# kakaoenterprise/JORLDY

Measured on NVIDIA H100. Metric: env_steps_per_sec, higher is better.
Workload: dtype f32

## Files before the change

include/jorldy_b200.h:

```cpp
#ifndef JORLDY_B200_H
#define JORLDY_B200_H

#include <stdint.h>

#ifdef __cplusplus
#define JB_API extern "C"
#else
#define JB_API
#endif

JB_API int jb_env_classic_reset(int kind, double* phys, float* obs, int32_t* elapsed, int64_t* episode,
                                float* score, const uint8_t* mask, uint64_t seed, uint64_t stream_base,
                                int n, void* stream);
JB_API int jb_env_classic_step(int kind, double* phys, float* obs, int32_t* elapsed, int64_t* episode,
                               float* score, const void* action, int action_kind, float* next_obs,
                               float* reward, float* done, float* stats, int auto_reset, int max_steps,
                               uint64_t seed, uint64_t stream_base, int n, void* stream);

JB_API int jb_gae(const float* reward, const float* done, const float* value, const float* next_value,
                  const float* last_value, int N, int T, float gamma, float lambda, int standardize,
                  float* adv, float* ret, void* stream);

JB_API int
jb_env_synth_reset(float* obs, int32_t* elapsed, int64_t* episode, float* score, uint64_t seed,
// ... 41 lines not shown
                            const float* relu_act, void* stream);
JB_API int jb_linear_bwd_dw(const float* dy, const float* x, float* dw, float* db, int M, int in_f, int out_f,
                            void* stream);
JB_API int
jb_linear_bwd_dw_splitk(const float* dy, const float* x, float* dw, float* db, int M, int in_f, int out_f,
                        float* workspace, int splits, void* stream);
JB_API int jb_linear_io_fwd(const float* x, const float* w, const float* b, float* y, int M, int in_f, int out_f,
                            int relu, void* stream);
JB_API int jb_linear_io_bwd_dx(const float* dy, const float* w, float* dx, int M, int in_f, int out_f,
                               const float* relu_act, void* stream);
JB_API int jb_linear_io_bwd_dw(const float* dy, const float* x, float* dw, int M, int in_f, int out_f, void* stream);
JB_API int jb_colsum(const float* x, int M, int N, float* out, int accumulate, void* stream);
JB_API int jb_mlp_in_fwd(const float* x, const int32_t* idx, const float* w1, const float* b1, int M, int D, int H,
                         float* h1, float* xg, void* stream);
JB_API int jb_heads_fwd(const float* h, int M, int H, const float* w0, const float* b0, int n0, const float* w1,
                        const float* b1, int n1, const float* w2, const float* b2, int n2, float* out, void* stream);
JB_API int jb_heads_bwd_dx(const float* dout, const float* h, int M, int H, const float* w0, int n0, const float* w1,
                           int n1, const float* w2, int n2, float* dh, void* stream);
JB_API int jb_heads_bwd_dw(const float* dout, const float* h, int M, int H, float* dw0, float* db0, int n0, float* dw1,
                           float* db1, int n1, float* dw2, float* db2, int n2, void* stream);

JB_API int jb_ppo_act_discrete(const float* out, int M, int A, int nout, const float* u, uint64_t seed,
                               uint64_t stream_base, uint64_t ctr, long long* row_ctr, int greedy, int64_t* action,
                               void* stream);
JB_API int jb_ppo_act_continuous(const float* out, int M, int A, int nout, const float* normal, uint64_t seed,
                                 uint64_t stream_base, uint64_t ctr, long long* row_ctr, int greedy, float* action,
                                 void* stream);
JB_API int jb_ppo_prepass_discrete(const float* out, const int32_t* action, int M, int A, int nout, float* value,
                                   float* logp_old, void* stream);
JB_API int jb_ppo_prepass_continuous(const float* out, const float* action, int M, int A, int nout, float* value,
                                     float* logp_old, void* stream);
JB_API int jb_take_minibatch(const int32_t* perm, long long* cursor, int B, int32_t* cur_idx, void* stream);
JB_API int jb_ppo_loss(int continuous, const float* out, const int32_t* idx, const void* action, const float* adv,
                       const float* ret, const float* value_old, const float* logp_old, int B, int A, int nout,
                       float eps_clip, float vf_coef, float ent_coef, float* dout, float* stats, float* acc,
                       void* stream);

JB_API int jb_env_frames_reset(uint8_t* obs, int64_t* fcount, float* score, uint64_t seed, uint64_t stream_base, int n,
                               void* stream);
JB_API int jb_env_frames_step(uint8_t* obs, int64_t* fcount, float* score, uint8_t* next_obs, float* reward, float* done,
// ... 103 lines not shown
```

jorldy_b200/core/agent/ppo.py:

```python
import numpy as np
import torch

from ..buffer import FrameRollout, RolloutBuffer
from ..dev import C, ptr, require_cuda, stream_ptr
from ..network import Network
from ..optimizer import Optimizer
from .base import BaseAgent

GRAPH_CHUNK = 16
MAX_ACTION_SIZE = {"discrete": 18, "continuous": 8}


class PPO(BaseAgent):
    def __init__(
        self,
        state_size,
        action_size,
        hidden_size=512,
        network="discrete_policy_value",
        head="mlp",
        optim_config={"name": "adam"},
        gamma=0.99,
        use_standardization=True,
        run_step=1e6,
# ... 45 lines not shown

        self.seed = int(seed)
        self.rng_stream_base = 0
        self._row_ctr = {}
        self.use_cuda_graph = use_cuda_graph
        self.use_fused = use_fused
        self._fused = {}
        self._graphs = {}
        self._acc = torch.zeros(8, dtype=torch.float32, device=self.device)
        self._cursor = torch.zeros(1, dtype=torch.int64, device=self.device)
        self.world_size = 1
        self.allreduce = None
        self._inject_perms = None
        self.n_launches = 0
        self.n_prepass_launches = 0

    @property
    def continuous(self):
        return self.action_type == "continuous"

    def act_device(self, state, training=True, noise=None):
        net = self.network
        M = state.shape[0]
        out = net._buf("act.out", (M, net.nout))
        net.forward_rows(state, out)
        A = self.action_size
        row_ctr = self._row_ctr.get(M)
        if row_ctr is None:
            row_ctr = self._row_ctr[M] = torch.zeros(M, dtype=torch.int64, device=self.device)
        if self.continuous:
            action = net._buf("act.a", (M, A))
            C.jb_ppo_act_continuous(ptr(out), M, A, net.nout, ptr(noise), self.seed, self.rng_stream_base,
                                    0, ptr(row_ctr), int(not training), ptr(action), stream_ptr())
        else:
            action = net._buf("act.a", (M,), torch.int64)
            C.jb_ppo_act_discrete(ptr(out), M, A, net.nout, ptr(noise), self.seed, self.rng_stream_base,
                                  0, ptr(row_ctr), int(not training), ptr(action), stream_ptr())
        return action

    @torch.no_grad()
    def act(self, state, training=True):
        self.network.train(training)
        s = self.as_tensor(state)
        action = self.act_device(s.view(s.shape[0], -1), training)
        a = action.cpu().numpy()
        return {"action": a.reshape(a.shape[0], -1)}

    def _minibatch_step(self, st, idx, B):
        net = self.network
        tag = f"mb{B}."
        out = net.forward_raw(st["state"], idx, B, tag=tag)
        dout = net._buf(tag + "dout", (B, net.nout))
        stats = net._buf(tag + "stats", (8 + 4 * ((B + 255) // 256),))
        C.jb_ppo_loss(int(self.continuous), ptr(out), ptr(idx), ptr(st["action"]), ptr(st["adv"]), ptr(st["ret"]),
                      ptr(st["value"]), ptr(st["logp_old"]), B, self.action_size, net.nout, self.epsilon_clip,
                      self.vf_coef, self.ent_coef, ptr(dout), ptr(stats), ptr(self._acc), stream_ptr())
        net.backward_raw(dout, B, tag=tag)
        if self.allreduce is not None:
            self.allreduce(net.grad)
        self.optimizer.step(max_norm=self.clip_grad_norm)

# ... 17 lines not shown
        side = torch.cuda.Stream()
        side.wait_stream(torch.cuda.current_stream())
        with torch.cuda.stream(side):
            C.jb_take_minibatch(ptr(st["perm"]), ptr(self._cursor), B, ptr(cur_idx), stream_ptr())
            self._minibatch_step(st, cur_idx, B)
        torch.cuda.current_stream().wait_stream(side)
        torch.cuda.synchronize()
        for dst, src in zip(mutated, saved):
            dst.copy_(src)
        graph = torch.cuda.CUDAGraph()
        with torch.cuda.graph(graph):
            chunk()
        self._graphs[key] = graph
        return graph

    def _learn_tensors(self, state, action, reward, done, next_state=None, last_next_state=None):
        net = self.network
        NT = state.shape[0]
        T = self.n_step
        N = NT // T
        assert N * T == NT, f"rollout of {NT} rows is not a multiple of n_step={T} (ppo.py:97 view(-1, n_step) would raise)"
        A = self.action_size
        dev = self.device
        s = stream_ptr()
        st = getattr(self, "_st", None)
        if st is None or st["NT"] != NT:
            st = {"NT": NT,
                  "out": torch.empty(NT, net.nout, device=dev),
                  "value": torch.empty(NT, device=dev),
                  "logp_old": torch.empty(NT, A if self.continuous else 1, device=dev),
                  "adv": torch.empty(NT, device=dev), "ret": torch.empty(NT, device=dev),
                  "next_value": torch.empty(NT, device=dev),
                  "perm": torch.empty(NT, dtype=torch.int32, device=dev)}
            self._st = st
        st["state"] = state
        st["action"] = action
        net.forward_rows(state, st["out"])
        if self.continuous:
            C.jb_ppo_prepass_continuous(ptr(st["out"]), ptr(action), NT, A, net.nout, ptr(st["value"]),
                                        ptr(st["logp_old"]), s)
        else:
            C.jb_ppo_prepass_discrete(ptr(st["out"]), ptr(action), NT, A, net.nout, ptr(st["value"]),
                                      ptr(st["logp_old"]), s)
        if next_state is not None:
            nout = net._buf("next.out", (NT, net.nout))
            net.forward_rows(next_state, nout)
            st["next_value"].copy_(nout[:, -1])
            nv, lv = st["next_value"], None
        else:
            lout = net._buf("last.out", (N, net.nout))
            net.forward_rows(last_next_state, lout)
            lv = net._buf("last.v", (N,))
            lv.copy_(lout[:, -1])
            nv = None
        C.jb_gae(ptr(reward), ptr(done), ptr(st["value"]), ptr(nv), ptr(lv), N, T, self.gamma, self._lambda,
                 int(self.use_standardization), ptr(st["adv"]), ptr(st["ret"]), s)
        mean_ret = st["ret"].mean()

        B = self.batch_size
        self.optimizer._sync_lr()
        self._acc.zero_()
        self._acc[3] = -float("inf")
        self._acc[4] = float("inf")
        n_full = NT // B
        tail = NT - n_full * B
        from . import ppo_fused
        use_fused = self.use_fused and n_full > 0 and ppo_fused.supported(self, B)
        if use_fused and B not in self._fused:
            self._fused[B] = ppo_fused.FusedRunner(self, B)
        use_graph = (not use_fused) and self.use_cuda_graph and n_full >= GRAPH_CHUNK
        n_steps = 0
        for epoch in range(self.n_epoch):
            if self._inject_perms is not None:
                perm = torch.as_tensor(np.asarray(self._inject_perms[epoch]), dtype=torch.int32, device=dev)
            else:
                perm = torch.randperm(NT, device=dev, dtype=torch.int32)
            st["perm"].copy_(perm)
            self._cursor.zero_()
            done_steps = 0
            if use_fused:
                self._fused[B].run(st, n_full)
                done_steps = n_full
            if use_graph:
                g = self._graph_for(st, B)
                for _ in range(n_full // GRAPH_CHUNK):
                    g.replay()
                done_steps = (n_full // GRAPH_CHUNK) * GRAPH_CHUNK
            for k in range(done_steps, n_full):
                self._minibatch_step(st, st["perm"][k * B:(k + 1) * B], B)
            if tail:
                self._minibatch_step(st, st["perm"][n_full * B:], tail)
            n_steps += n_full + (1 if tail else 0)
        self.n_launches = (self.n_epoch * (1 + (self.LAUNCHES_PER_MINIBATCH if tail else 0)) if use_fused
                           else n_steps * self.LAUNCHES_PER_MINIBATCH)
        n_chunks = (NT + 16383) // 16384
        self.n_prepass_launches = 3 * n_chunks + 1 + 3 + 1

        acc = torch.cat([self._acc[:6], mean_ret.view(1), self._acc[7:8]]).cpu().numpy()
        if acc[7] != 0.0:
            dbg = [ws["partials"][200:205].tolist() for ws in (r.ws for r in self._fused.values())]
            raise RuntimeError("persistent PPO kernel: a peer GPU did not reach the gradient exchange (flag wait timed out); "
                               f"[kind 1=grad-ready 2=done-reading, peer, step, seen, target] = {dbg}")
        cnt = max(acc[5], 1.0)
        return {
            "actor_loss": float(acc[0] / cnt),
            "critic_loss": float(acc[1] / cnt),
            "entropy_loss": float(acc[2] / cnt),
            "max_ratio": float(acc[3]),
            "min_prob": float(acc[4]),
            "mean_ret": float(acc[6]),
        }

    def _action_to_device(self, action):
# ... 18 lines not shown
            self._host_in = hin
        hin["state"].copy_(torch.as_tensor(tr["state"], dtype=torch.float32, device=dev).reshape(n, -1))
        hin["next_state"].copy_(torch.as_tensor(tr["next_state"], dtype=torch.float32, device=dev).reshape(n, -1))
        hin["reward"].copy_(torch.as_tensor(tr["reward"], dtype=torch.float32, device=dev).reshape(-1))
        hin["done"].copy_(torch.as_tensor(tr["done"], dtype=torch.float32, device=dev).reshape(-1))
        hin["action"].copy_(self._action_to_device(tr["action"]))
        return self._learn_tensors(hin["state"], hin["action"], hin["reward"], hin["done"], next_state=hin["next_state"])

    def learn_rollout(self, rollout):
        N, T = rollout.N, rollout.T
        frames = isinstance(rollout, FrameRollout)
        if frames:
            state, last = rollout.rows(), rollout.last_rows()
        else:
            state, last = rollout.state.view(N * T, -1), rollout.last_next_state
        res = self._learn_tensors(state, rollout.action.view(N * T, -1) if self.continuous
                                  else rollout.action.view(N * T), rollout.reward.view(N * T),
                                  rollout.done.view(N * T), last_next_state=last)
        if frames:
            rollout.frames.check()
        rollout.clear()
        return res

    def process(self, transitions, step):
        result = {}
        self.memory.store(transitions)
        delta_t = step - self.time_t
        self.time_t = step
        self.learn_stamp += delta_t
        if self.learn_stamp >= self.n_step:
            result = self.learn()
            if self.lr_decay:
                self.learning_rate_decay(step)
# ... 3 lines not shown
```

jorldy_b200/core/buffer/rollout_buffer.py:

```python
import numpy as np
import torch

from ..dev import require_cuda
from .base import BaseBuffer
from .frame_store import FrameRows, FrameStore, frames_per_rollout


class RolloutBuffer(BaseBuffer):
    def __init__(self):
        super().__init__()
        self.buffer = list()

    def store(self, transitions):
        if self.first_store:
            self.check_dim(transitions[0])
        self.buffer += transitions

    def sample(self):
        transitions = self.stack_transition(self.buffer)
        self.buffer.clear()
        return transitions

    def sample_batched(self):
        out = {}
        for key in self.buffer[0].keys():
            arr = np.stack([np.asarray(b[key]) for b in self.buffer], axis=1)
            out[key] = arr.reshape((-1,) + arr.shape[2:])
        self.buffer.clear()
        return out

    @property
    def size(self):
        return len(self.buffer)


class DeviceRollout:
    def __init__(self, num_envs, n_step, state_size, action_size, action_type, device=None):
        dev = require_cuda(device)
        N, T = num_envs, n_step
        self.N, self.T, self.device = N, T, dev
        self.state = torch.zeros(N, T, state_size, dtype=torch.float32, device=dev)
        if action_type == "discrete":
            self.action = torch.zeros(N, T, dtype=torch.int32, device=dev)
        else:
            self.action = torch.zeros(N, T, action_size, dtype=torch.float32, device=dev)
        self.reward = torch.zeros(N, T, dtype=torch.float32, device=dev)
        self.done = torch.zeros(N, T, dtype=torch.float32, device=dev)
        self.last_next_state = torch.zeros(N, state_size, dtype=torch.float32, device=dev)
        self.t = 0

    def write(self, state, action, reward, done, next_state):
        t = self.t
        self.state[:, t].copy_(state)
        if self.action.dtype == torch.int32:
            self.action[:, t].copy_(action.view(self.N))
        else:
# ... 10 lines not shown
            self.action[:, t].copy_(action.view(self.N))
        else:
            self.action[:, t].copy_(action.view(self.N, -1))
        self.reward[:, t].copy_(reward)
        self.done[:, t].copy_(done)
        if t == self.T - 1:
            self.last_next_state.copy_(next_state)
        self.t = t + 1

    @property
    def full(self):
        return self.t >= self.T

    def clear(self):
        self.t = 0


class FrameRollout(DeviceRollout):

    def __init__(self, num_envs, n_step, action_size, action_type, device=None):
        dev = require_cuda(device)
        N, T = num_envs, n_step
        self.N, self.T, self.device = N, T, dev
        self.frames = FrameStore(N, frames_per_rollout(T), dev)
        self.state_ref = torch.zeros(N, T, dtype=torch.int64, device=dev)
        if action_type == "discrete":
            self.action = torch.zeros(N, T, dtype=torch.int32, device=dev)
        else:
            self.action = torch.zeros(N, T, action_size, dtype=torch.float32, device=dev)
        self.reward = torch.zeros(N, T, dtype=torch.float32, device=dev)
        self.done = torch.zeros(N, T, dtype=torch.float32, device=dev)
        self.last_next_state = torch.zeros(N, dtype=torch.int64, device=dev)
        self._refs = torch.zeros(2, N, dtype=torch.int64, device=dev)
        self.t = 0

    def start(self, obs):
        self.frames.start(obs)

    def push(self, obs, next_obs, done, auto_reset):
        s, x = self.frames.push(obs, next_obs, done, auto_reset, out=self._refs)
        self.state_ref[:, self.t].copy_(s)
        return x

    def rows(self):
        return FrameRows(self.frames, self.state_ref.view(-1))

    def last_rows(self):
        return FrameRows(self.frames, self.last_next_state)
# ... 1 lines not shown
```

jorldy_b200/core/collect.py:

```python
import torch

from .buffer import DeviceRollout, FrameRollout, frame_store


class RolloutCollector:
    def __init__(self, env, agent, n_step=None, use_cuda_graph=True):
        self.env, self.agent = env, agent
        self.T = n_step or agent.n_step
        self.frames = bool(getattr(env, "frame_stack", False))
        if self.frames:
            self.rollout = FrameRollout(env.num_envs, self.T, env.action_size, env.action_type, device=agent.device)
        else:
            self.rollout = DeviceRollout(env.num_envs, self.T, env.state_size, env.action_size, env.action_type,
                                         device=agent.device)
        self.use_cuda_graph = use_cuda_graph
        self._graph = None
        self.launches_per_collect = 5 * self.T
        env.reset_device()
        if self.frames:
            self.rollout.start(env.obs)

    def _collect_eager(self):
        env, agent, ro = self.env, self.agent, self.rollout
        ro.clear()
        for t in range(self.T):
            if not self.frames:
                ro.state[:, t].copy_(env.obs)
            action = agent.act_device(env.obs, training=True)
            next_obs, reward, done = env.step_device(action)
            ro.t = t
            if self.frames:
                next_obs = ro.push(env.obs, next_obs, done, env.auto_reset)
            ro.write_after_step(action, reward, done, next_obs)

    def collect(self):
        if not self.use_cuda_graph:
            self._collect_eager()
            return self.rollout
        if self._graph is None:
            side = torch.cuda.Stream()
            side.wait_stream(torch.cuda.current_stream())
            with torch.cuda.stream(side):
                self._collect_eager()
            torch.cuda.current_stream().wait_stream(side)
            torch.cuda.synchronize()
            g = torch.cuda.CUDAGraph()
            with torch.cuda.graph(g):
                self._collect_eager()
            self._graph = g
        self._graph.replay()
        self.rollout.t = self.T
        return self.rollout


class NStepAssembler:

    def __init__(self, n_step, apex=False, gamma=0.99):
        self.n, self.apex, self.gamma = n_step, apex, gamma
        self.L = n_step + 1 if apex else n_step
        self.hist, self.count, self.pos = None, 0, 0

    def push(self, tr):
        if self.hist is None:
            self.hist = {k: torch.zeros((v.shape[0], self.L) + tuple(v.shape[1:]), dtype=v.dtype, device=v.device)
                         for k, v in tr.items()}
        for k, v in tr.items():
            self.hist[k][:, self.pos].copy_(v)
# ... 68 lines not shown
```

jorldy_b200/core/network/base.py:

```python
from collections import OrderedDict

import torch

from ..dev import C, ptr, require_cuda, stream_ptr

MAX_ROWS_PER_PASS = 16384


def orthogonal_(shape, gain, generator=None):
    w = torch.empty(shape, dtype=torch.float32)
    torch.nn.init.orthogonal_(w, gain, generator=generator)
    return w


def init_gain(nonlinearity):
    if isinstance(nonlinearity, str):
        if nonlinearity == "policy":
            return 0.01
        return torch.nn.init.calculate_gain(nonlinearity)
    return float(nonlinearity)


class _ParamList(list):
    network = None


class FlatNetwork:

    def __init__(self, device=None):
        self.device = require_cuda(device)
        self._specs = []
        self.training = True
        self._ws = {}

    def _allocate(self):
        total, offs = 0, []
        for _, shape in self._specs:
            n = 1
            for s in shape:
                n *= s
            offs.append(total)
            total += (n + 3) // 4 * 4
        self.num_flat = total
        self.flat = torch.zeros(total, dtype=torch.float32, device=self.device)
        self.grad = torch.zeros(total, dtype=torch.float32, device=self.device)
        self._offs = offs
        self.p = OrderedDict()
        self.g = OrderedDict()
# ... 22 lines not shown
        params = _ParamList(self.p.values())
        params.network = self
        return params

    def state_dict(self):
        return OrderedDict((k, v.detach().clone()) for k, v in self.p.items())

    def load_state_dict(self, sd):
        missing = [k for k in self.p if k not in sd]
        extra = [k for k in sd if k not in self.p]
        if missing or extra:
            raise KeyError(f"state_dict mismatch: missing {missing}, unexpected {extra}")
        with torch.no_grad():
            for k, v in self.p.items():
                v.copy_(torch.as_tensor(sd[k], dtype=torch.float32).to(self.device).view_as(v))

    def copy_from(self, other):
        assert other.num_flat == self.num_flat
        C.jb_copy_f32(ptr(self.flat), ptr(other.flat), self.num_flat, stream_ptr())

    def train(self, mode=True):
        self.training = mode
        return self

    def to(self, device):
        return self

    def _buf(self, key, shape, dtype=torch.float32):
        k = (key, tuple(shape), dtype)
        t = self._ws.get(k)
        if t is None:
            t = torch.empty(*shape, dtype=dtype, device=self.device)
            self._ws[k] = t
        return t
# ... 1 lines not shown
```

jorldy_b200/core/network/layers.py:

```python
from ..dev import C, ptr, stream_ptr


import os

TC_MIN_ROWS = 1024
_USE_TC = os.environ.get("JB_NO_TC", "0") != "1"


def linear_fwd(x, w, b, y, relu):
    M, in_f = x.shape
    out_f = w.shape[0]
    if _USE_TC and M >= TC_MIN_ROWS and M % 128 == 0 and out_f % 128 == 0 and in_f % 32 == 0 and b is not None:
        C.jb_linear_fwd_tc(ptr(x), ptr(w), ptr(b), ptr(y), M, in_f, out_f, int(relu), stream_ptr())
        return
    C.jb_linear_fwd(ptr(x), ptr(w), ptr(b), ptr(y), M, in_f, out_f, int(relu), stream_ptr())


def linear_bwd_dx(dy, w, dx, relu_act=None, accumulate=False):
    M, out_f = dy.shape
    in_f = w.shape[1]
    if accumulate:
        C.jb_gemm(ptr(dy), out_f, 1, ptr(w), in_f, 0, ptr(dx), in_f, M, in_f, out_f, 0, 0,
                  ptr(relu_act), in_f, 0, 1, stream_ptr())
    else:
        C.jb_linear_bwd_dx(ptr(dy), ptr(w), ptr(dx), M, in_f, out_f, ptr(relu_act), stream_ptr())


# ... 13 lines not shown
    if accumulate:
        C.jb_gemm(ptr(dy), out_f, 1, ptr(w), out_f, 1, ptr(dx), in_f, M, in_f, out_f, 0, 0,
                  ptr(relu_act), in_f, 0, 1, stream_ptr())
    else:
        C.jb_linear_io_bwd_dx(ptr(dy), ptr(w), ptr(dx), M, in_f, out_f, ptr(relu_act), stream_ptr())


def linear_io_bwd_dw(dy, x, dw, db):
    M, out_f = dy.shape
    C.jb_linear_io_bwd_dw(ptr(dy), ptr(x), ptr(dw), M, x.shape[1], out_f, stream_ptr())
    C.jb_colsum(ptr(dy), M, out_f, ptr(db), 0, stream_ptr())


def heads_fwd(h, heads, out):
    M, H = h.shape
    a = []
    for i in range(3):
        if i < len(heads):
            w, b = heads[i]
            a += [ptr(w), ptr(b), w.shape[0]]
        else:
            a += [0, 0, 0]
    C.jb_heads_fwd(ptr(h), M, H, *a, ptr(out), stream_ptr())


def heads_bwd_dx(dout, h, heads, dh):
    M, H = h.shape
    a = []
    for i in range(3):
        if i < len(heads):
            a += [ptr(heads[i][0]), heads[i][0].shape[0]]
        else:
            a += [0, 0]
    C.jb_heads_bwd_dx(ptr(dout), ptr(h), M, H, *a, ptr(dh), stream_ptr())


def heads_bwd_dw(dout, h, grads):
    M, H = h.shape
# ... 9 lines not shown
```

jorldy_b200/core/network/policy_value.py:

```python
import torch

from .base import FlatNetwork, init_gain, orthogonal_
from .head import make_head
from . import layers as L


class _PolicyValue(FlatNetwork):
    head_names = ()

    def __init__(self, D_in, D_out, D_hidden=512, head="mlp", device=None, seed=None):
        super().__init__(device)
        self.D_in, self.D_out, self.D_hidden = D_in, D_out, D_hidden
        self.head = make_head(head, D_in, D_hidden)
        self.out_heads = self._out_heads(D_out)
        self.nout = sum(n for _, n, _ in self.out_heads)
        self._wide = self.nout > 32
        assert not self._wide or len(self.out_heads) == 1
        specs = self.head.specs() + [("l.weight", (D_hidden, self.head.D_head_out)), ("l.bias", (D_hidden,))]
        for name, n, _ in self.out_heads:
            specs += [(f"{name}.weight", (n, D_hidden)), (f"{name}.bias", (n,))]
        self._specs = specs
        self._allocate()
        gen = torch.Generator().manual_seed(seed) if seed is not None else None
        with torch.no_grad():
# ... 17 lines not shown
            out = self._buf(tag + "out", (M, self.nout))
        if self._wide:
            w, b = self._heads_wb()[0]
            L.linear_fwd(h2, w, b, out, relu=False)
        else:
            L.heads_fwd(h2, self._heads_wb(), out)
        return out

    def forward_rows(self, x, out):
        M = x.shape[0]
        for s in range(0, M, self.head.max_rows):
            e = min(M, s + self.head.max_rows)
            self.forward_raw(x[s:e], None, e - s, out[s:e], tag=f"inf{e - s}.", save=False)
        return out

    def backward_raw(self, dout, M, tag="t."):
        h1 = self._buf(tag + "head.h", (M, self.head.D_head_out))
        h2 = self._buf(tag + "h2", (M, self.D_hidden))
        dh2 = self._buf(tag + "dh2", (M, self.D_hidden))
        dh1 = self._buf(tag + "dh1", (M, self.head.D_head_out))
        if self._wide:
            (w, _), (dw, db) = self._heads_wb()[0], self._heads_grads()[0]
            L.linear_bwd_dw(dout, h2, dw, db)
            L.linear_bwd_dx(dout, w, dh2, relu_act=h2)
        else:
            L.heads_bwd_dw(dout, h2, self._heads_grads())
            L.heads_bwd_dx(dout, h2, self._heads_wb(), dh2)
        L.linear_bwd_dw(dh2, h1, self.g["l.weight"], self.g["l.bias"])
        L.linear_bwd_dx(dh2, self.p["l.weight"], dh1, relu_act=h1)
        self.head.backward(self, dh1, M, tag)
# ... 23 lines not shown
```

jorldy_b200/core/optimizer/__init__.py:

```python
from collections import OrderedDict

import numpy as np
import torch

from ..dev import C, ptr, stream_ptr


class _FlatOptimizer:
    def __init__(self, params, lr):
        net = getattr(params, "network", None)
        if net is None:
            raise TypeError("jorldy_b200 optimizers take `params=network.parameters()` of a FlatNetwork")
        self.network = net
        self.defaults = {"lr": lr}
        self.param_groups = [{"lr": lr, "params": list(range(len(net.p)))}]
        dev = net.device
        self._lr_dev = torch.tensor([lr], dtype=torch.float32, device=dev)
        self._lr_host = float(lr)
        self._step_dev = torch.zeros(1, dtype=torch.int64, device=dev)
        self._n_partials = C.jb_grad_partials_count(net.num_flat)
        self._partials = torch.zeros(self._n_partials, dtype=torch.float32, device=dev)
        self.grad_norm = torch.zeros(1, dtype=torch.float32, device=dev)

    def _sync_lr(self):
# ... 21 lines not shown

    def __init__(self, params, lr=1e-3, betas=(0.9, 0.999), eps=1e-8, **kwargs):
        super().__init__(params, lr)
        self.betas, self.eps = betas, eps
        self.exp_avg = torch.zeros_like(self.network.flat)
        self.exp_avg_sq = torch.zeros_like(self.network.flat)

    def step(self, max_norm=None):
        self._sync_lr()
        net, s = self.network, stream_ptr()
        C.jb_grad_sumsq(ptr(net.grad), net.num_flat, ptr(self._partials), ptr(self._step_dev), s)
        C.jb_adam_step(ptr(net.flat), ptr(net.grad), ptr(self.exp_avg), ptr(self.exp_avg_sq), net.num_flat,
                       ptr(self._lr_dev), self.betas[0], self.betas[1], self.eps, ptr(self._step_dev),
                       ptr(self._partials), self._n_partials, float(max_norm) if max_norm else 0.0,
                       ptr(self.grad_norm), s)

    def state_dict(self):
        step = float(self._step_dev.item())
        m, v = self._slot_views(self.exp_avg), self._slot_views(self.exp_avg_sq)
        state = {i: {"step": torch.tensor(step), "exp_avg": m[i].clone(), "exp_avg_sq": v[i].clone()}
                 for i in range(len(m))} if step > 0 else {}
        group = {"lr": float(self.param_groups[0]["lr"]), "betas": self.betas, "eps": self.eps, "weight_decay": 0,
                 "amsgrad": False, "params": list(range(len(m)))}
        return {"state": state, "param_groups": [group]}

    def load_state_dict(self, sd):
        g = sd["param_groups"][0]
        self.param_groups[0]["lr"] = float(g["lr"])
        st = sd.get("state", {})
        if st:
# ... 12 lines not shown
    def __init__(self, params, lr=1e-2, alpha=0.99, eps=1e-8, centered=False, **kwargs):
        super().__init__(params, lr)
        if not centered:
            raise NotImplementedError("only RMSprop(centered=True) is on the hot path (config/ape_x/*.py)")
        self.alpha, self.eps, self.centered = alpha, eps, centered
        self.square_avg = torch.zeros_like(self.network.flat)
        self.grad_avg = torch.zeros_like(self.network.flat)

    def step(self, max_norm=None):
        self._sync_lr()
        net, s = self.network, stream_ptr()
        C.jb_grad_sumsq(ptr(net.grad), net.num_flat, ptr(self._partials), ptr(self._step_dev), s)
        C.jb_rmsprop_centered_step(ptr(net.flat), ptr(net.grad), ptr(self.square_avg), ptr(self.grad_avg),
                                   net.num_flat, ptr(self._lr_dev), self.alpha, self.eps, ptr(self._partials),
                                   self._n_partials, float(max_norm) if max_norm else 0.0, ptr(self.grad_norm), s)

    def state_dict(self):
        step = float(self._step_dev.item())
        sq, ga = self._slot_views(self.square_avg), self._slot_views(self.grad_avg)
        state = {i: {"step": torch.tensor(step), "square_avg": sq[i].clone(), "grad_avg": ga[i].clone()}
                 for i in range(len(sq))} if step > 0 else {}
        group = {"lr": float(self.param_groups[0]["lr"]), "alpha": self.alpha, "eps": self.eps, "centered": True,
                 "momentum": 0, "weight_decay": 0, "params": list(range(len(sq)))}
        return {"state": state, "param_groups": [group]}

    def load_state_dict(self, sd):
        self.param_groups[0]["lr"] = float(sd["param_groups"][0]["lr"])
        st = sd.get("state", {})
        if st:
            sq, ga = self._slot_views(self.square_avg), self._slot_views(self.grad_avg)
# ... 22 lines not shown
```

jorldy_b200/csrc/heads.cu:

```cuda
#include "common.cuh"

namespace {

constexpr int MAX_DIN = 32;
constexpr int MAX_NOUT = 32;

__global__ void mlp_in_fwd_kernel(const float* __restrict__ x, const int32_t* __restrict__ idx,
                                  const float* __restrict__ W1, const float* __restrict__ b1,
                                  int M, int D, int H, float* __restrict__ h1, float* __restrict__ xg) {
  const int m = blockIdx.y;
  const int j = blockIdx.x * blockDim.x + threadIdx.x;
  __shared__ float sx[MAX_DIN];
  const int row = idx ? idx[m] : m;
  if (threadIdx.x < D) {
    const float v = x[(size_t)row * D + threadIdx.x];
    sx[threadIdx.x] = v;
    if (xg && blockIdx.x == 0) xg[(size_t)m * D + threadIdx.x] = v;
  }
  __syncthreads();
  if (j >= H) return;
  float acc = 0.f;
  for (int i = 0; i < D; ++i) acc = fmaf(sx[i], W1[(size_t)j * D + i], acc);
  acc += b1[j];
  h1[(size_t)m * H + j] = fmaxf(acc, 0.f);
}

struct HeadRows {
  const float* w[MAX_NOUT];
  const float* b[MAX_NOUT];
};
struct HeadGradRows {
  float* dw[MAX_NOUT];
  float* db[MAX_NOUT];
};

__global__ void __launch_bounds__(256)
heads_fwd_kernel(const float* __restrict__ h, int M, int H, HeadRows hr, int nout, float* __restrict__ out) {
  const int warp = (blockIdx.x * blockDim.x + threadIdx.x) >> 5;
  const int lane = threadIdx.x & 31;
  if (warp >= M) return;
  float acc[MAX_NOUT];
#pragma unroll
  for (int o = 0; o < MAX_NOUT; ++o) acc[o] = 0.f;
  const float* hrow = h + (size_t)warp * H;
  int j = lane;
  for (; j + 96 < H; j += 128) {
    float hv[4];
#pragma unroll
    for (int u = 0; u < 4; ++u) hv[u] = hrow[j + 32 * u];
#pragma unroll
    for (int o = 0; o < MAX_NOUT; ++o) {
      if (o < nout) {
        float wv[4];
#pragma unroll
        for (int u = 0; u < 4; ++u) wv[u] = hr.w[o][j + 32 * u];
#pragma unroll
        for (int u = 0; u < 4; ++u) acc[o] = fmaf(hv[u], wv[u], acc[o]);
      }
    }
  }
  for (; j < H; j += 32) {
    const float hv = hrow[j];
#pragma unroll
    for (int o = 0; o < MAX_NOUT; ++o)
      if (o < nout) acc[o] = fmaf(hv, hr.w[o][j], acc[o]);
  }
#pragma unroll
  for (int o = 0; o < MAX_NOUT; ++o) {
    if (o < nout) {
      const float v = jb_warp_sum(acc[o]);
      if (lane == 0) out[(size_t)warp * nout + o] = v + *hr.b[o];
    }
  }
}

__global__ void heads_bwd_dx_kernel(const float* __restrict__ dout, const float* __restrict__ h, int M, int H,
                                    HeadRows hr, int nout, float* __restrict__ dh) {
  const int m = blockIdx.y;
  const int j = blockIdx.x * blockDim.x + threadIdx.x;
  __shared__ float sd[MAX_NOUT];
  if (threadIdx.x < nout) sd[threadIdx.x] = dout[(size_t)m * nout + threadIdx.x];
  __syncthreads();
  if (j >= H) return;
  float acc = 0.f;
#pragma unroll
  for (int o = 0; o < MAX_NOUT; ++o)
// ... 63 lines not shown
  for (int g = 0; g < 3; ++g)
    for (int q = 0; q < n[g]; ++q, ++o) {
      if (o >= MAX_NOUT || !w[g]) return false;
      hr.w[o] = w[g] + (size_t)q * H;
      hr.b[o] = b[g] ? b[g] + q : nullptr;
    }
  for (; o < MAX_NOUT; ++o) { hr.w[o] = nullptr; hr.b[o] = nullptr; }
  return true;
}

}

JB_API int jb_mlp_in_fwd(const float* x, const int32_t* idx, const float* w1, const float* b1, int M, int D, int H,
                         float* h1, float* xg, void* stream) {
  if (!x || !w1 || !b1 || !h1 || M <= 0 || D <= 0 || D > MAX_DIN || H <= 0) return JB_ERR_INVALID;
  dim3 grid(jb_div_up(H, 128), M);
  mlp_in_fwd_kernel<<<grid, 128, 0, (cudaStream_t)stream>>>(x, idx, w1, b1, M, D, H, h1, xg);
  return jb_check_launch();
}

JB_API int jb_heads_fwd(const float* h, int M, int H, const float* w0, const float* b0, int n0, const float* w1,
                        const float* b1, int n1, const float* w2, const float* b2, int n2, float* out, void* stream) {
  const int nout = n0 + n1 + n2;
  if (!h || !out || M <= 0 || H <= 0 || nout <= 0 || nout > MAX_NOUT) return JB_ERR_INVALID;
  const float* w[3] = {w0, w1, w2}; const float* b[3] = {b0, b1, b2}; const int n[3] = {n0, n1, n2};
  for (int g = 0; g < 3; ++g) if (n[g] > 0 && (!w[g] || !b[g])) return JB_ERR_INVALID;
  HeadRows hr;
  if (!fill_rows(hr, w, b, n, H)) return JB_ERR_INVALID;
  const int threads = 256;
  heads_fwd_kernel<<<jb_div_up((long long)M * 32, threads), threads, 0, (cudaStream_t)stream>>>(h, M, H, hr, nout, out);
  return jb_check_launch();
}

JB_API int jb_heads_bwd_dx(const float* dout, const float* h, int M, int H, const float* w0, int n0, const float* w1,
                           int n1, const float* w2, int n2, float* dh, void* stream) {
  const int nout = n0 + n1 + n2;
  if (!dout || !h || !dh || M <= 0 || H <= 0 || nout <= 0 || nout > MAX_NOUT) return JB_ERR_INVALID;
  const float* w[3] = {w0, w1, w2}; const float* b[3] = {nullptr, nullptr, nullptr}; const int n[3] = {n0, n1, n2};
  HeadRows hr;
  if (!fill_rows(hr, w, b, n, H)) return JB_ERR_INVALID;
  dim3 grid(jb_div_up(H, 128), M);
  heads_bwd_dx_kernel<<<grid, 128, 0, (cudaStream_t)stream>>>(dout, h, M, H, hr, nout, dh);
  return jb_check_launch();
}

// ... 18 lines not shown
```

jorldy_b200/csrc/ppo.cu:

```cuda
#include "common.cuh"
#include "philox.cuh"
#include "ppo_rowmath.cuh"

namespace {

using jbppo::MAX_A;
using jbppo::MAX_A_DISC;
using jbppo::log_softmax_row;
using jbppo::atanh_clamped;

template <int NA>
__global__ void ppo_act_discrete_kernel(const float* __restrict__ out, int M, int A, int nout,
                                        const float* __restrict__ u_in, uint64_t seed, uint64_t stream_base,
                                        uint64_t ctr, long long* __restrict__ row_ctr, int greedy,
                                        int64_t* __restrict__ action) {
  const int m = blockIdx.x * blockDim.x + threadIdx.x;
  if (m >= M) return;
  if (row_ctr) { ctr += (uint64_t)row_ctr[m]; row_ctr[m] += 1; }
  float lg[NA], lsm[NA];
#pragma unroll
  for (int a = 0; a < NA; ++a) lg[a] = a < A ? out[(size_t)m * nout + a] : 0.f;
  log_softmax_row<NA>(lg, A, lsm);
  int pick = 0;
  if (greedy) {
    float best = expf(lsm[0]);
#pragma unroll
    for (int a = 1; a < NA; ++a) if (a < A) { const float p = expf(lsm[a]); if (p > best) { best = p; pick = a; } }
  } else {
    float u;
    if (u_in) u = u_in[m];
    else { jb_philox4 r = jb_philox(seed, stream_base + (uint64_t)m, ctr); u = jb_u01_float(r.x); }
    float tot = 0.f;
#pragma unroll
    for (int a = 0; a < NA; ++a) if (a < A) tot += expf(lsm[a]);
    const float target = u * tot;
    float c = 0.f;
    bool found = false;
    pick = A - 1;
#pragma unroll
    for (int a = 0; a < NA; ++a) if (a < A && !found) { c += expf(lsm[a]); if (target < c) { pick = a; found = true; } }
  }
  action[m] = pick;
}

__global__ void ppo_act_continuous_kernel(const float* __restrict__ out, int M, int A, int nout,
                                          const float* __restrict__ n_in, uint64_t seed, uint64_t stream_base,
                                          uint64_t ctr, long long* __restrict__ row_ctr, int greedy,
                                          float* __restrict__ action) {
  const int m = blockIdx.x * blockDim.x + threadIdx.x;
  if (m >= M) return;
  if (row_ctr) { ctr += (uint64_t)row_ctr[m]; row_ctr[m] += 1; }
  for (int a = 0; a < A; a += 2) {
    float n0 = 0.f, n1 = 0.f;
    if (!greedy) {
      if (n_in) { n0 = n_in[(size_t)m * A + a]; if (a + 1 < A) n1 = n_in[(size_t)m * A + a + 1]; }
      else {
        jb_philox4 r = jb_philox(seed, stream_base + (uint64_t)m, ctr * 8 + (uint64_t)(a >> 1));
        const float u1 = (float)((r.x >> 8) + 1u) * (1.0f / 16777216.0f);
        const float u2 = jb_u01_float(r.y);
        const float rad = sqrtf(-2.0f * logf(u1));
        n0 = rad * cospif(2.0f * u2); n1 = rad * sinpif(2.0f * u2);
      }
    }
    for (int q = 0; q < 2 && a + q < A; ++q) {
      const float mu = fminf(fmaxf(out[(size_t)m * nout + a + q], -5.f), 5.f);
      const float sd = expf(tanhf(out[(size_t)m * nout + A + a + q]));
      const float z = greedy ? mu : fmaf(sd, q ? n1 : n0, mu);
      action[(size_t)m * A + a + q] = tanhf(z);
    }
  }
}

template <int NA>
__global__ void ppo_prepass_discrete_kernel(const float* __restrict__ out, const int32_t* __restrict__ action,
                                            int M, int A, int nout, float* __restrict__ value,
                                            float* __restrict__ logp_old) {
  const int m = blockIdx.x * blockDim.x + threadIdx.x;
  if (m >= M) return;
  float lg[NA], lsm[NA];
#pragma unroll
  for (int a = 0; a < NA; ++a) lg[a] = a < A ? out[(size_t)m * nout + a] : 0.f;
// ... 119 lines not shown
                                      int32_t* __restrict__ cur_idx) {
  const long long base = (*cursor) * (long long)B;
  for (int i = threadIdx.x; i < B; i += blockDim.x) cur_idx[i] = perm[base + i];
  __syncthreads();
  if (threadIdx.x == 0) *cursor += 1;
}

}

JB_API int jb_take_minibatch(const int32_t* perm, long long* cursor, int B, int32_t* cur_idx, void* stream) {
  if (!perm || !cursor || !cur_idx || B <= 0) return JB_ERR_INVALID;
  take_minibatch_kernel<<<1, 256, 0, (cudaStream_t)stream>>>(perm, cursor, B, cur_idx);
  return jb_check_launch();
}

JB_API int jb_ppo_act_discrete(const float* out, int M, int A, int nout, const float* u, uint64_t seed,
                               uint64_t stream_base, uint64_t ctr, long long* row_ctr, int greedy, int64_t* action,
                               void* stream) {
  if (!out || !action || M <= 0 || A <= 0 || A > MAX_A_DISC || nout < A) return JB_ERR_INVALID;
  const dim3 grid(jb_div_up(M, 128));
  cudaStream_t s = (cudaStream_t)stream;
  if (A <= MAX_A) ppo_act_discrete_kernel<MAX_A><<<grid, 128, 0, s>>>(out, M, A, nout, u, seed, stream_base, ctr, row_ctr, greedy, action);
  else ppo_act_discrete_kernel<MAX_A_DISC><<<grid, 128, 0, s>>>(out, M, A, nout, u, seed, stream_base, ctr, row_ctr, greedy, action);
  return jb_check_launch();
}

JB_API int jb_ppo_act_continuous(const float* out, int M, int A, int nout, const float* normal, uint64_t seed,
                                 uint64_t stream_base, uint64_t ctr, long long* row_ctr, int greedy, float* action,
                                 void* stream) {
  if (!out || !action || M <= 0 || A <= 0 || A > MAX_A || nout < 2 * A) return JB_ERR_INVALID;
  ppo_act_continuous_kernel<<<jb_div_up(M, 128), 128, 0, (cudaStream_t)stream>>>(out, M, A, nout, normal, seed, stream_base, ctr, row_ctr, greedy, action);
  return jb_check_launch();
}

JB_API int jb_ppo_prepass_discrete(const float* out, const int32_t* action, int M, int A, int nout, float* value,
                                   float* logp_old, void* stream) {
  if (!out || !action || !value || !logp_old || M <= 0 || A <= 0 || A > MAX_A_DISC || nout != A + 1) return JB_ERR_INVALID;
  const dim3 grid(jb_div_up(M, 128));
  cudaStream_t s = (cudaStream_t)stream;
  if (A <= MAX_A) ppo_prepass_discrete_kernel<MAX_A><<<grid, 128, 0, s>>>(out, action, M, A, nout, value, logp_old);
  else ppo_prepass_discrete_kernel<MAX_A_DISC><<<grid, 128, 0, s>>>(out, action, M, A, nout, value, logp_old);
  return jb_check_launch();
}

JB_API int jb_ppo_prepass_continuous(const float* out, const float* action, int M, int A, int nout, float* value,
                                     float* logp_old, void* stream) {
// ... 21 lines not shown
```

Baseline: 1.825 million.

## Reuse rollout policy outputs in PPO prepass and retile input/head kernels

During collection the policy outputs from acting are written straight into a rollout buffer through a strided output, and a network version counter records which weights produced them. At learn time, if the weights are unchanged and the row counts give bitwise-identical kernel paths, the prepass forward over all N*T states is skipped. The input-layer kernel now handles 16 rows per block with weights held in registers, and the heads kernel gains a 512-wide unrolled loop. The cost is extra rollout memory and version bookkeeping, and the reused outputs are only valid while the row-exactness check holds.

```diff
diff --git a/include/jorldy_b200.h b/include/jorldy_b200.h
--- a/include/jorldy_b200.h
+++ b/include/jorldy_b200.h
@@ -79,16 +79,17 @@
 JB_API int jb_mlp_in_fwd(const float* x, const int32_t* idx, const float* w1, const float* b1, int M, int D, int H,
                          float* h1, float* xg, void* stream);
 JB_API int jb_heads_fwd(const float* h, int M, int H, const float* w0, const float* b0, int n0, const float* w1,
-                        const float* b1, int n1, const float* w2, const float* b2, int n2, float* out, void* stream);
+                        const float* b1, int n1, const float* w2, const float* b2, int n2, float* out, int ldo,
+                        void* stream);
 JB_API int jb_heads_bwd_dx(const float* dout, const float* h, int M, int H, const float* w0, int n0, const float* w1,
                            int n1, const float* w2, int n2, float* dh, void* stream);
 JB_API int jb_heads_bwd_dw(const float* dout, const float* h, int M, int H, float* dw0, float* db0, int n0, float* dw1,
                            float* db1, int n1, float* dw2, float* db2, int n2, void* stream);
 
-JB_API int jb_ppo_act_discrete(const float* out, int M, int A, int nout, const float* u, uint64_t seed,
+JB_API int jb_ppo_act_discrete(const float* out, int M, int A, int ldo, const float* u, uint64_t seed,
                                uint64_t stream_base, uint64_t ctr, long long* row_ctr, int greedy, int64_t* action,
                                void* stream);
-JB_API int jb_ppo_act_continuous(const float* out, int M, int A, int nout, const float* normal, uint64_t seed,
+JB_API int jb_ppo_act_continuous(const float* out, int M, int A, int ldo, const float* normal, uint64_t seed,
                                  uint64_t stream_base, uint64_t ctr, long long* row_ctr, int greedy, float* action,
                                  void* stream);
 JB_API int jb_ppo_prepass_discrete(const float* out, const int32_t* action, int M, int A, int nout, float* value,
diff --git a/jorldy_b200/core/agent/ppo.py b/jorldy_b200/core/agent/ppo.py
--- a/jorldy_b200/core/agent/ppo.py
+++ b/jorldy_b200/core/agent/ppo.py
@@ -83,15 +83,17 @@
         self._inject_perms = None
         self.n_launches = 0
         self.n_prepass_launches = 0
+        self.timeline = None
 
     @property
     def continuous(self):
         return self.action_type == "continuous"
 
-    def act_device(self, state, training=True, noise=None):
+    def act_device(self, state, training=True, noise=None, out=None):
         net = self.network
         M = state.shape[0]
-        out = net._buf("act.out", (M, net.nout))
+        if out is None:
+            out = net._buf("act.out", (M, net.nout))
         net.forward_rows(state, out)
         A = self.action_size
         row_ctr = self._row_ctr.get(M)
@@ -99,11 +101,11 @@
             row_ctr = self._row_ctr[M] = torch.zeros(M, dtype=torch.int64, device=self.device)
         if self.continuous:
             action = net._buf("act.a", (M, A))
-            C.jb_ppo_act_continuous(ptr(out), M, A, net.nout, ptr(noise), self.seed, self.rng_stream_base,
+            C.jb_ppo_act_continuous(ptr(out), M, A, out.stride(0), ptr(noise), self.seed, self.rng_stream_base,
                                     0, ptr(row_ctr), int(not training), ptr(action), stream_ptr())
         else:
             action = net._buf("act.a", (M,), torch.int64)
-            C.jb_ppo_act_discrete(ptr(out), M, A, net.nout, ptr(noise), self.seed, self.rng_stream_base,
+            C.jb_ppo_act_discrete(ptr(out), M, A, out.stride(0), ptr(noise), self.seed, self.rng_stream_base,
                                   0, ptr(row_ctr), int(not training), ptr(action), stream_ptr())
         return action
 
@@ -114,6 +116,12 @@
         action = self.act_device(s.view(s.shape[0], -1), training)
         a = action.cpu().numpy()
         return {"action": a.reshape(a.shape[0], -1)}
+
+    def _mark(self, piece):
+        if self.timeline is not None:
+            ev = torch.cuda.Event(enable_timing=True)
+            ev.record()
+            self.timeline.append((piece, ev))
 
     def _minibatch_step(self, st, idx, B):
         net = self.network
@@ -161,7 +169,7 @@
         self._graphs[key] = graph
         return graph
 
-    def _learn_tensors(self, state, action, reward, done, next_state=None, last_next_state=None):
+    def _learn_tensors(self, state, action, reward, done, next_state=None, last_next_state=None, out=None):
         net = self.network
         NT = state.shape[0]
         T = self.n_step
@@ -182,12 +190,17 @@
             self._st = st
         st["state"] = state
         st["action"] = action
-        net.forward_rows(state, st["out"])
+        self._mark("start")
+        prepass_forward = out is None
+        if prepass_forward:
+            out = st["out"]
+            net.forward_rows(state, out)
+            self._mark("prepass_forward")
         if self.continuous:
-            C.jb_ppo_prepass_continuous(ptr(st["out"]), ptr(action), NT, A, net.nout, ptr(st["value"]),
+            C.jb_ppo_prepass_continuous(ptr(out), ptr(action), NT, A, net.nout, ptr(st["value"]),
                                         ptr(st["logp_old"]), s)
         else:
-            C.jb_ppo_prepass_discrete(ptr(st["out"]), ptr(action), NT, A, net.nout, ptr(st["value"]),
+            C.jb_ppo_prepass_discrete(ptr(out), ptr(action), NT, A, net.nout, ptr(st["value"]),
                                       ptr(st["logp_old"]), s)
         if next_state is not None:
             nout = net._buf("next.out", (NT, net.nout))
@@ -203,6 +216,7 @@
         C.jb_gae(ptr(reward), ptr(done), ptr(st["value"]), ptr(nv), ptr(lv), N, T, self.gamma, self._lambda,
                  int(self.use_standardization), ptr(st["adv"]), ptr(st["ret"]), s)
         mean_ret = st["ret"].mean()
+        self._mark("prepass_gae")
 
         B = self.batch_size
         self.optimizer._sync_lr()
@@ -224,6 +238,7 @@
                 perm = torch.randperm(NT, device=dev, dtype=torch.int32)
             st["perm"].copy_(perm)
             self._cursor.zero_()
+            self._mark("perm")
             done_steps = 0
             if use_fused:
                 self._fused[B].run(st, n_full)
@@ -238,12 +253,15 @@
             if tail:
                 self._minibatch_step(st, st["perm"][n_full * B:], tail)
             n_steps += n_full + (1 if tail else 0)
+            self._mark("epoch")
+        net.version += 1
         self.n_launches = (self.n_epoch * (1 + (self.LAUNCHES_PER_MINIBATCH if tail else 0)) if use_fused
                            else n_steps * self.LAUNCHES_PER_MINIBATCH)
-        n_chunks = (NT + 16383) // 16384
-        self.n_prepass_launches = 3 * n_chunks + 1 + 3 + 1
+        n_chunks = (NT + net.head.max_rows - 1) // net.head.max_rows
+        self.n_prepass_launches = 3 * n_chunks * prepass_forward + 1 + 3 + 1
 
         acc = torch.cat([self._acc[:6], mean_ret.view(1), self._acc[7:8]]).cpu().numpy()
+        self._mark("readback")
         if acc[7] != 0.0:
             dbg = [ws["partials"][200:205].tolist() for ws in (r.ws for r in self._fused.values())]
             raise RuntimeError("persistent PPO kernel: a peer GPU did not reach the gradient exchange (flag wait timed out); "
@@ -292,9 +310,14 @@
             state, last = rollout.rows(), rollout.last_rows()
         else:
             state, last = rollout.state.view(N * T, -1), rollout.last_next_state
+        net = self.network
+        out = None
+        if (rollout.out is not None and rollout.out_version == (net, net.version) and net.rows_exact(N)
+                and net.rows_exact(N * T)):
+            out = rollout.out.view(N * T, net.nout)
         res = self._learn_tensors(state, rollout.action.view(N * T, -1) if self.continuous
                                   else rollout.action.view(N * T), rollout.reward.view(N * T),
-                                  rollout.done.view(N * T), last_next_state=last)
+                                  rollout.done.view(N * T), last_next_state=last, out=out)
         if frames:
             rollout.frames.check()
         rollout.clear()
diff --git a/jorldy_b200/core/buffer/rollout_buffer.py b/jorldy_b200/core/buffer/rollout_buffer.py
--- a/jorldy_b200/core/buffer/rollout_buffer.py
+++ b/jorldy_b200/core/buffer/rollout_buffer.py
@@ -35,11 +35,13 @@
 
 
 class DeviceRollout:
-    def __init__(self, num_envs, n_step, state_size, action_size, action_type, device=None):
+    def __init__(self, num_envs, n_step, state_size, action_size, action_type, device=None, nout=None):
         dev = require_cuda(device)
         N, T = num_envs, n_step
         self.N, self.T, self.device = N, T, dev
         self.state = torch.zeros(N, T, state_size, dtype=torch.float32, device=dev)
+        self.out = torch.zeros(N, T, nout, dtype=torch.float32, device=dev) if nout else None
+        self.out_version = None
         if action_type == "discrete":
             self.action = torch.zeros(N, T, dtype=torch.int32, device=dev)
         else:
@@ -80,6 +82,7 @@
 
     def clear(self):
         self.t = 0
+        self.out_version = None
 
 
 class FrameRollout(DeviceRollout):
@@ -98,6 +101,7 @@
         self.done = torch.zeros(N, T, dtype=torch.float32, device=dev)
         self.last_next_state = torch.zeros(N, dtype=torch.int64, device=dev)
         self._refs = torch.zeros(2, N, dtype=torch.int64, device=dev)
+        self.out, self.out_version = None, None
         self.t = 0
 
     def start(self, obs):
diff --git a/jorldy_b200/core/collect.py b/jorldy_b200/core/collect.py
--- a/jorldy_b200/core/collect.py
+++ b/jorldy_b200/core/collect.py
@@ -12,7 +12,7 @@
             self.rollout = FrameRollout(env.num_envs, self.T, env.action_size, env.action_type, device=agent.device)
         else:
             self.rollout = DeviceRollout(env.num_envs, self.T, env.state_size, env.action_size, env.action_type,
-                                         device=agent.device)
+                                         device=agent.device, nout=agent.network.nout)
         self.use_cuda_graph = use_cuda_graph
         self._graph = None
         self.launches_per_collect = 5 * self.T
@@ -26,7 +26,7 @@
         for t in range(self.T):
             if not self.frames:
                 ro.state[:, t].copy_(env.obs)
-            action = agent.act_device(env.obs, training=True)
+            action = agent.act_device(env.obs, training=True, out=None if self.frames else ro.out[:, t])
             next_obs, reward, done = env.step_device(action)
             ro.t = t
             if self.frames:
@@ -36,6 +36,7 @@
     def collect(self):
         if not self.use_cuda_graph:
             self._collect_eager()
+            self._stamp()
             return self.rollout
         if self._graph is None:
             side = torch.cuda.Stream()
@@ -50,7 +51,13 @@
             self._graph = g
         self._graph.replay()
         self.rollout.t = self.T
+        self._stamp()
         return self.rollout
+
+    def _stamp(self):
+        net = self.agent.network
+        if self.rollout.out is not None:
+            self.rollout.out_version = (net, net.version)
 
 
 class NStepAssembler:
diff --git a/jorldy_b200/core/network/base.py b/jorldy_b200/core/network/base.py
--- a/jorldy_b200/core/network/base.py
+++ b/jorldy_b200/core/network/base.py
@@ -32,6 +32,7 @@
         self._specs = []
         self.training = True
         self._ws = {}
+        self.version = 0
 
     def _allocate(self):
         total, offs = 0, []
@@ -84,10 +85,12 @@
         with torch.no_grad():
             for k, v in self.p.items():
                 v.copy_(torch.as_tensor(sd[k], dtype=torch.float32).to(self.device).view_as(v))
+        self.version += 1
 
     def copy_from(self, other):
         assert other.num_flat == self.num_flat
         C.jb_copy_f32(ptr(self.flat), ptr(other.flat), self.num_flat, stream_ptr())
+        self.version += 1
 
     def train(self, mode=True):
         self.training = mode
diff --git a/jorldy_b200/core/network/layers.py b/jorldy_b200/core/network/layers.py
--- a/jorldy_b200/core/network/layers.py
+++ b/jorldy_b200/core/network/layers.py
@@ -7,10 +7,14 @@
 _USE_TC = os.environ.get("JB_NO_TC", "0") != "1"
 
 
+def uses_tc(M, in_f, out_f):
+    return _USE_TC and M >= TC_MIN_ROWS and M % 128 == 0 and out_f % 128 == 0 and in_f % 32 == 0
+
+
 def linear_fwd(x, w, b, y, relu):
     M, in_f = x.shape
     out_f = w.shape[0]
-    if _USE_TC and M >= TC_MIN_ROWS and M % 128 == 0 and out_f % 128 == 0 and in_f % 32 == 0 and b is not None:
+    if uses_tc(M, in_f, out_f) and b is not None:
         C.jb_linear_fwd_tc(ptr(x), ptr(w), ptr(b), ptr(y), M, in_f, out_f, int(relu), stream_ptr())
         return
     C.jb_linear_fwd(ptr(x), ptr(w), ptr(b), ptr(y), M, in_f, out_f, int(relu), stream_ptr())
@@ -54,6 +58,7 @@
 
 def heads_fwd(h, heads, out):
     M, H = h.shape
+    assert out.stride(1) == 1
     a = []
     for i in range(3):
         if i < len(heads):
@@ -61,7 +66,7 @@
             a += [ptr(w), ptr(b), w.shape[0]]
         else:
             a += [0, 0, 0]
-    C.jb_heads_fwd(ptr(h), M, H, *a, ptr(out), stream_ptr())
+    C.jb_heads_fwd(ptr(h), M, H, *a, ptr(out), out.stride(0), stream_ptr())
 
 
 def heads_bwd_dx(dout, h, heads, dh):
diff --git a/jorldy_b200/core/network/policy_value.py b/jorldy_b200/core/network/policy_value.py
--- a/jorldy_b200/core/network/policy_value.py
+++ b/jorldy_b200/core/network/policy_value.py
@@ -55,6 +55,12 @@
             self.forward_raw(x[s:e], None, e - s, out[s:e], tag=f"inf{e - s}.", save=False)
         return out
 
+    def rows_exact(self, M):
+        if self.head.kind != "mlp" or self._wide:
+            return False
+        step = self.head.max_rows
+        return all(L.uses_tc(m, self.head.D_head_out, self.D_hidden) for m in {min(M, step), M % step or min(M, step)})
+
     def backward_raw(self, dout, M, tag="t."):
         h1 = self._buf(tag + "head.h", (M, self.head.D_head_out))
         h2 = self._buf(tag + "h2", (M, self.D_hidden))
diff --git a/jorldy_b200/core/optimizer/__init__.py b/jorldy_b200/core/optimizer/__init__.py
--- a/jorldy_b200/core/optimizer/__init__.py
+++ b/jorldy_b200/core/optimizer/__init__.py
@@ -59,6 +59,7 @@
                        ptr(self._lr_dev), self.betas[0], self.betas[1], self.eps, ptr(self._step_dev),
                        ptr(self._partials), self._n_partials, float(max_norm) if max_norm else 0.0,
                        ptr(self.grad_norm), s)
+        net.version += 1
 
     def state_dict(self):
         step = float(self._step_dev.item())
@@ -101,6 +102,7 @@
         C.jb_rmsprop_centered_step(ptr(net.flat), ptr(net.grad), ptr(self.square_avg), ptr(self.grad_avg),
                                    net.num_flat, ptr(self._lr_dev), self.alpha, self.eps, ptr(self._partials),
                                    self._n_partials, float(max_norm) if max_norm else 0.0, ptr(self.grad_norm), s)
+        net.version += 1
 
     def state_dict(self):
         step = float(self._step_dev.item())
diff --git a/jorldy_b200/csrc/heads.cu b/jorldy_b200/csrc/heads.cu
--- a/jorldy_b200/csrc/heads.cu
+++ b/jorldy_b200/csrc/heads.cu
@@ -5,24 +5,34 @@
 constexpr int MAX_DIN = 32;
 constexpr int MAX_NOUT = 32;
 
-__global__ void mlp_in_fwd_kernel(const float* __restrict__ x, const int32_t* __restrict__ idx,
-                                  const float* __restrict__ W1, const float* __restrict__ b1,
-                                  int M, int D, int H, float* __restrict__ h1, float* __restrict__ xg) {
-  const int m = blockIdx.y;
+constexpr int IN_ROWS = 16;
+__global__ void __launch_bounds__(128)
+mlp_in_fwd_kernel(const float* __restrict__ x, const int32_t* __restrict__ idx, const float* __restrict__ W1,
+                  const float* __restrict__ b1, int M, int D, int H, float* __restrict__ h1, float* __restrict__ xg) {
+  const int m0 = blockIdx.y * IN_ROWS;
+  const int nr = min(IN_ROWS, M - m0);
   const int j = blockIdx.x * blockDim.x + threadIdx.x;
-  __shared__ float sx[MAX_DIN];
-  const int row = idx ? idx[m] : m;
-  if (threadIdx.x < D) {
-    const float v = x[(size_t)row * D + threadIdx.x];
-    sx[threadIdx.x] = v;
-    if (xg && blockIdx.x == 0) xg[(size_t)m * D + threadIdx.x] = v;
+  __shared__ float sx[IN_ROWS][MAX_DIN];
+  for (int e = threadIdx.x; e < nr * D; e += blockDim.x) {
+    const int r = e / D, i = e - r * D;
+    const int row = idx ? idx[m0 + r] : m0 + r;
+    const float v = x[(size_t)row * D + i];
+    sx[r][i] = v;
+    if (xg && blockIdx.x == 0) xg[(size_t)(m0 + r) * D + i] = v;
   }
   __syncthreads();
   if (j >= H) return;
-  float acc = 0.f;
-  for (int i = 0; i < D; ++i) acc = fmaf(sx[i], W1[(size_t)j * D + i], acc);
-  acc += b1[j];
-  h1[(size_t)m * H + j] = fmaxf(acc, 0.f);
+  float w[MAX_DIN];
+#pragma unroll
+  for (int i = 0; i < MAX_DIN; ++i) w[i] = i < D ? W1[(size_t)j * D + i] : 0.f;
+  const float bj = b1[j];
+  for (int r = 0; r < nr; ++r) {
+    float acc = 0.f;
+#pragma unroll
+    for (int i = 0; i < MAX_DIN; ++i) if (i < D) acc = fmaf(sx[r][i], w[i], acc);
+    acc += bj;
+    h1[(size_t)(m0 + r) * H + j] = fmaxf(acc, 0.f);
+  }
 }
 
 struct HeadRows {
@@ -35,7 +45,7 @@
 };
 
 __global__ void __launch_bounds__(256)
-heads_fwd_kernel(const float* __restrict__ h, int M, int H, HeadRows hr, int nout, float* __restrict__ out) {
+heads_fwd_kernel(const float* __restrict__ h, int M, int H, HeadRows hr, int nout, float* __restrict__ out, int ldo) {
   const int warp = (blockIdx.x * blockDim.x + threadIdx.x) >> 5;
   const int lane = threadIdx.x & 31;
   if (warp >= M) return;
@@ -44,6 +54,21 @@
   for (int o = 0; o < MAX_NOUT; ++o) acc[o] = 0.f;
   const float* hrow = h + (size_t)warp * H;
   int j = lane;
+  for (; j + 480 < H; j += 512) {
+    float hv[16];
+#pragma unroll
+    for (int u = 0; u < 16; ++u) hv[u] = hrow[j + 32 * u];
+#pragma unroll
+    for (int o = 0; o < MAX_NOUT; ++o) {
+      if (o < nout) {
+        float wv[16];
+#pragma unroll
+        for (int u = 0; u < 16; ++u) wv[u] = hr.w[o][j + 32 * u];
+#pragma unroll
+        for (int u = 0; u < 16; ++u) acc[o] = fmaf(hv[u], wv[u], acc[o]);
+      }
+    }
+  }
   for (; j + 96 < H; j += 128) {
     float hv[4];
 #pragma unroll
@@ -69,7 +94,7 @@
   for (int o = 0; o < MAX_NOUT; ++o) {
     if (o < nout) {
       const float v = jb_warp_sum(acc[o]);
-      if (lane == 0) out[(size_t)warp * nout + o] = v + *hr.b[o];
+      if (lane == 0) out[(size_t)warp * ldo + o] = v + *hr.b[o];
     }
   }
 }
@@ -163,21 +188,22 @@
 JB_API int jb_mlp_in_fwd(const float* x, const int32_t* idx, const float* w1, const float* b1, int M, int D, int H,
                          float* h1, float* xg, void* stream) {
   if (!x || !w1 || !b1 || !h1 || M <= 0 || D <= 0 || D > MAX_DIN || H <= 0) return JB_ERR_INVALID;
-  dim3 grid(jb_div_up(H, 128), M);
+  dim3 grid(jb_div_up(H, 128), jb_div_up(M, IN_ROWS));
   mlp_in_fwd_kernel<<<grid, 128, 0, (cudaStream_t)stream>>>(x, idx, w1, b1, M, D, H, h1, xg);
   return jb_check_launch();
 }
 
 JB_API int jb_heads_fwd(const float* h, int M, int H, const float* w0, const float* b0, int n0, const float* w1,
-                        const float* b1, int n1, const float* w2, const float* b2, int n2, float* out, void* stream) {
+                        const float* b1, int n1, const float* w2, const float* b2, int n2, float* out, int ldo,
+                        void* stream) {
   const int nout = n0 + n1 + n2;
-  if (!h || !out || M <= 0 || H <= 0 || nout <= 0 || nout > MAX_NOUT) return JB_ERR_INVALID;
+  if (!h || !out || M <= 0 || H <= 0 || nout <= 0 || nout > MAX_NOUT || ldo < nout) return JB_ERR_INVALID;
   const float* w[3] = {w0, w1, w2}; const float* b[3] = {b0, b1, b2}; const int n[3] = {n0, n1, n2};
   for (int g = 0; g < 3; ++g) if (n[g] > 0 && (!w[g] || !b[g])) return JB_ERR_INVALID;
   HeadRows hr;
   if (!fill_rows(hr, w, b, n, H)) return JB_ERR_INVALID;
   const int threads = 256;
-  heads_fwd_kernel<<<jb_div_up((long long)M * 32, threads), threads, 0, (cudaStream_t)stream>>>(h, M, H, hr, nout, out);
+  heads_fwd_kernel<<<jb_div_up((long long)M * 32, threads), threads, 0, (cudaStream_t)stream>>>(h, M, H, hr, nout, out, ldo);
   return jb_check_launch();
 }
 
diff --git a/jorldy_b200/csrc/ppo.cu b/jorldy_b200/csrc/ppo.cu
--- a/jorldy_b200/csrc/ppo.cu
+++ b/jorldy_b200/csrc/ppo.cu
@@ -10,7 +10,7 @@
 using jbppo::atanh_clamped;
 
 template <int NA>
-__global__ void ppo_act_discrete_kernel(const float* __restrict__ out, int M, int A, int nout,
+__global__ void ppo_act_discrete_kernel(const float* __restrict__ out, int M, int A, int ldo,
                                         const float* __restrict__ u_in, uint64_t seed, uint64_t stream_base,
                                         uint64_t ctr, long long* __restrict__ row_ctr, int greedy,
                                         int64_t* __restrict__ action) {
@@ -19,7 +19,7 @@
   if (row_ctr) { ctr += (uint64_t)row_ctr[m]; row_ctr[m] += 1; }
   float lg[NA], lsm[NA];
 #pragma unroll
-  for (int a = 0; a < NA; ++a) lg[a] = a < A ? out[(size_t)m * nout + a] : 0.f;
+  for (int a = 0; a < NA; ++a) lg[a] = a < A ? out[(size_t)m * ldo + a] : 0.f;
   log_softmax_row<NA>(lg, A, lsm);
   int pick = 0;
   if (greedy) {
@@ -43,7 +43,7 @@
   action[m] = pick;
 }
 
-__global__ void ppo_act_continuous_kernel(const float* __restrict__ out, int M, int A, int nout,
+__global__ void ppo_act_continuous_kernel(const float* __restrict__ out, int M, int A, int ldo,
                                           const float* __restrict__ n_in, uint64_t seed, uint64_t stream_base,
                                           uint64_t ctr, long long* __restrict__ row_ctr, int greedy,
                                           float* __restrict__ action) {
@@ -63,8 +63,8 @@
       }
     }
     for (int q = 0; q < 2 && a + q < A; ++q) {
-      const float mu = fminf(fmaxf(out[(size_t)m * nout + a + q], -5.f), 5.f);
-      const float sd = expf(tanhf(out[(size_t)m * nout + A + a + q]));
+      const float mu = fminf(fmaxf(out[(size_t)m * ldo + a + q], -5.f), 5.f);
+      const float sd = expf(tanhf(out[(size_t)m * ldo + A + a + q]));
       const float z = greedy ? mu : fmaf(sd, q ? n1 : n0, mu);
       action[(size_t)m * A + a + q] = tanhf(z);
     }
@@ -214,22 +214,22 @@
   return jb_check_launch();
 }
 
-JB_API int jb_ppo_act_discrete(const float* out, int M, int A, int nout, const float* u, uint64_t seed,
+JB_API int jb_ppo_act_discrete(const float* out, int M, int A, int ldo, const float* u, uint64_t seed,
                                uint64_t stream_base, uint64_t ctr, long long* row_ctr, int greedy, int64_t* action,
                                void* stream) {
-  if (!out || !action || M <= 0 || A <= 0 || A > MAX_A_DISC || nout < A) return JB_ERR_INVALID;
+  if (!out || !action || M <= 0 || A <= 0 || A > MAX_A_DISC || ldo < A) return JB_ERR_INVALID;
   const dim3 grid(jb_div_up(M, 128));
   cudaStream_t s = (cudaStream_t)stream;
-  if (A <= MAX_A) ppo_act_discrete_kernel<MAX_A><<<grid, 128, 0, s>>>(out, M, A, nout, u, seed, stream_base, ctr, row_ctr, greedy, action);
-  else ppo_act_discrete_kernel<MAX_A_DISC><<<grid, 128, 0, s>>>(out, M, A, nout, u, seed, stream_base, ctr, row_ctr, greedy, action);
-  return jb_check_launch();
-}
-
-JB_API int jb_ppo_act_continuous(const float* out, int M, int A, int nout, const float* normal, uint64_t seed,
+  if (A <= MAX_A) ppo_act_discrete_kernel<MAX_A><<<grid, 128, 0, s>>>(out, M, A, ldo, u, seed, stream_base, ctr, row_ctr, greedy, action);
+  else ppo_act_discrete_kernel<MAX_A_DISC><<<grid, 128, 0, s>>>(out, M, A, ldo, u, seed, stream_base, ctr, row_ctr, greedy, action);
+  return jb_check_launch();
+}
+
+JB_API int jb_ppo_act_continuous(const float* out, int M, int A, int ldo, const float* normal, uint64_t seed,
                                  uint64_t stream_base, uint64_t ctr, long long* row_ctr, int greedy, float* action,
                                  void* stream) {
-  if (!out || !action || M <= 0 || A <= 0 || A > MAX_A || nout < 2 * A) return JB_ERR_INVALID;
-  ppo_act_continuous_kernel<<<jb_div_up(M, 128), 128, 0, (cudaStream_t)stream>>>(out, M, A, nout, normal, seed, stream_base, ctr, row_ctr, greedy, action);
+  if (!out || !action || M <= 0 || A <= 0 || A > MAX_A || ldo < 2 * A) return JB_ERR_INVALID;
+  ppo_act_continuous_kernel<<<jb_div_up(M, 128), 128, 0, (cudaStream_t)stream>>>(out, M, A, ldo, normal, seed, stream_base, ctr, row_ctr, greedy, action);
   return jb_check_launch();
 }
 
```

Measured after the change: 1.864 million (median of 6 runs). 1.02x the previous value.
